# ChuhanZhou/News_Recommendation_Model

Hardware: AMD Instinct MI355X
Metric: train impressions/sec (higher is better)
Workload: dtype f32

## Files before the change

news_recommendation_model_amd/csrc/common.hpp:

```cpp
#pragma once
#include <hip/hip_runtime.h>
#include <stdint.h>

namespace nrm {

using f32x4 = __attribute__((ext_vector_type(4))) float;
using u32x4 = __attribute__((ext_vector_type(4))) unsigned;
using bf16x8 = __attribute__((ext_vector_type(8))) __bf16;

constexpr int WAVE = 64;

inline int device_cus() {
    int dev = 0, cus = 256;
    if (hipGetDevice(&dev) != hipSuccess || hipDeviceGetAttribute(&cus, hipDeviceAttributeMultiprocessorCount, dev) != hipSuccess) cus = 256;
    return cus > 0 ? cus : 256;
}

__device__ __forceinline__ f32x4 mfma16(float a, float b, f32x4 c) {
    return __builtin_amdgcn_mfma_f32_16x16x4f32(a, b, c, 0, 0, 0);
}

struct GeluParts { float cdf; float e; };
__device__ __forceinline__ GeluParts gelu_parts(float x) {
    const float a = fabsf(x) * 0.70710678118654752440f;
    const float t = __builtin_amdgcn_rcpf(fmaf(0.3275911f, a, 1.0f));
    const float e = __builtin_amdgcn_exp2f(-1.44269504088896340736f * a * a);
    float poly = fmaf(1.061405429f, t, -1.453152027f);
    poly = fmaf(poly, t, 1.421413741f);
    poly = fmaf(poly, t, -0.284496736f);
    poly = fmaf(poly, t, 0.254829592f);
    const float half_erfc = 0.5f * poly * t * e;
    GeluParts r;
    r.cdf = x >= 0.f ? 1.0f - half_erfc : half_erfc;
    r.e = e;
    return r;
// ... 61 lines not shown
    v += __shfl_xor(v, 8);
    return v;
}

__device__ __forceinline__ float sum_rows4(float v) {
    const auto a = __builtin_amdgcn_permlane16_swap(__float_as_uint(v), __float_as_uint(v), false, false);
    const float y = __uint_as_float(a[0]) + __uint_as_float(a[1]);
    const auto b = __builtin_amdgcn_permlane32_swap(__float_as_uint(y), __float_as_uint(y), false, false);
    return __uint_as_float(b[0]) + __uint_as_float(b[1]);
}

__device__ __forceinline__ float wave_sum64(float v) {
    v = wave_sum16(v);
    v += __shfl_xor(v, 16);
    v += __shfl_xor(v, 32);
    return v;
}

__device__ __forceinline__ void store_b128_guarded(u32x4 v, __amdgpu_buffer_rsrc_t rs, unsigned voffset, int soffset) {
#if defined(__HIP_DEVICE_COMPILE__)
    __builtin_amdgcn_raw_buffer_store_b128(v, rs, voffset, soffset, 0);
#if !defined(NRM_STORE_GUARD) || NRM_STORE_GUARD == 2
    __builtin_amdgcn_sched_barrier(0);
    asm volatile("s_nop 3");
    __builtin_amdgcn_sched_barrier(0);
#elif NRM_STORE_GUARD == 1
    asm volatile("s_nop 3");
#endif
#endif
}

__host__ __device__ inline int swz4(int row) { return ((row >> 3) & 1) * 3; }

}
```

news_recommendation_model_amd/csrc/gemm.hip:

```cpp
#include <cstdlib>
#include <type_traits>
#include "common.hpp"
#include "gemm.hpp"
#ifndef NRM_PRIO
#define NRM_PRIO 0
#endif
#ifndef NRM_DIAG_GEMM
#define NRM_DIAG_GEMM 0
#endif

namespace nrm {

__global__ void pack_rows_kernel(const float* __restrict__ src, long rs, long cs, int nrows, int ncols,
                                 int rows, int kchunks, float* __restrict__ packed) {
    const long total = (long)kchunks * rows * 16;
    for (long i = (long)blockIdx.x * blockDim.x + threadIdx.x; i < total; i += (long)gridDim.x * blockDim.x) {
        const int j = (int)(i & 15);
        const long rc = i >> 4;
        const int row = (int)(rc % rows);
        const int c = (int)(rc / rows);
        const int slot = (j >> 2) ^ swz4(row);
        const int col = c * 16 + 4 * slot + (j & 3);
        packed[i] = (row < nrows && col < ncols) ? src[row * rs + col * cs] : 0.0f;
    }
}

__global__ __launch_bounds__(256) void pack_rows_multi_kernel(const PackTable tab) {
    const PackEntry e = tab.e[blockIdx.y];
    if (e.fmt) {
        const int nimg = e.fmt;
        const long total = (long)(e.rows / 16) * e.kchunks * 512;
        __bf16* dst = reinterpret_cast<__bf16*>(e.dst);
        for (long i = (long)blockIdx.x * blockDim.x + threadIdx.x; i < total; i += (long)gridDim.x * blockDim.x) {
            const int j = (int)(i & 31), r16 = (int)((i >> 5) & 15);
            const long tc = i >> 9;
            const int c = (int)(tc % e.kchunks), it = (int)(tc / e.kchunks);
            const int n = 16 * it + r16, k = 32 * c + j;
            float v = 0.0f;
            if (n < e.nrows && k < e.ncols) {
                const long o = n * e.rs + k * e.cs;
                v = e.src[o];
// ... 11 lines not shown
        const int j = (int)(i & 15);
        const long rc = i >> 4;
        const int row = (int)(rc % e.rows);
        const int c = (int)(rc / e.rows);
        const int slot = (j >> 2) ^ swz4(row);
        const int col = c * 16 + 4 * slot + (j & 3);
        float v = 0.0f;
        if (row < e.nrows && col < e.ncols) {
            const long o = row * e.rs + col * e.cs;
            v = e.src[o];
            if (e.src2) v = fmaf(e.sign2, e.src2[o], v);
        }
        e.dst[i] = v;
    }
}

hipError_t pack_rows_multi_launch(const PackTable& tab, int n, long max_total, hipStream_t st) {
    if (n <= 0) return hipSuccess;
    long bx = (max_total + 255) / 256;
    if (bx > 128) bx = 128;
    if (bx < 1) bx = 1;
    hipLaunchKernelGGL(pack_rows_multi_kernel, dim3((unsigned)bx, (unsigned)n), dim3(256), 0, st, tab);
    return hipGetLastError();
}

hipError_t pack_rows_launch(const float* src, long rs, long cs, int nrows, int ncols, int rows, int kchunks,
                            float* packed, hipStream_t st) {
    const long total = (long)kchunks * rows * 16;
    const int blocks = (int)((total + 255) / 256 > 4096 ? 4096 : (total + 255) / 256);
    hipLaunchKernelGGL(pack_rows_kernel, dim3(blocks), dim3(256), 0, st, src, rs, cs, nrows, ncols, rows, kchunks, packed);
    return hipGetLastError();
}

template <int NT, int MT, int EPI, int WPE = 2, int KC = 1>
__global__ __launch_bounds__(256, WPE) void gemm_nt_kernel(const GemmNtParams p) {
#if defined(__HIP_DEVICE_COMPILE__)
    constexpr int BM = 4 * MT * 16;
    constexpr int WROWS = NT * 16;
    constexpr int SUB = (WROWS + BM) * 16;
    constexpr int BUF = KC * SUB;
    __shared__ __attribute__((aligned(16))) float smem[2 * BUF];

    const int tid = threadIdx.x;
    const int lane = tid & 63;
    const int wave = __builtin_amdgcn_readfirstlane(tid >> 6);
    const int r16 = lane & 15, q = lane >> 4;
    const int M = p.M;
    const int m0 = blockIdx.x * BM;
    const int nc = blockIdx.y;
    const int n0 = nc * WROWS;

    constexpr unsigned OOB = 0x80000000u;
    const int rows_here = min(BM, M - m0);
    const __amdgpu_buffer_rsrc_t rs_w = __builtin_amdgcn_make_buffer_rsrc(const_cast<float*>(p.wp), 0, p.wp_bytes, 0x00020000);
    const __amdgpu_buffer_rsrc_t rs_x = __builtin_amdgcn_make_buffer_rsrc(
        const_cast<float*>(p.x) + (size_t)m0 * p.ldx, 0, ((rows_here - 1) * p.ldx + p.xcols) * 4, 0x00020000);
    const __amdgpu_buffer_rsrc_t rs_y = __builtin_amdgcn_make_buffer_rsrc(p.y + (size_t)m0 * p.ldy, 0, rows_here * p.ldy * 4, 0x00020000);
    const __amdgpu_buffer_rsrc_t rs_z = __builtin_amdgcn_make_buffer_rsrc(
        p.z ? p.z + (size_t)m0 * p.ldz : nullptr, 0, p.z ? rows_here * p.ldz * 4 : 0, 0x00020000);
    const __amdgpu_buffer_rsrc_t rs_b = __builtin_amdgcn_make_buffer_rsrc(const_cast<float*>(p.bias), 0, p.bias ? (p.N + 3) / 4 * 16 : 0, 0x00020000);
    const __amdgpu_buffer_rsrc_t rs_m = __builtin_amdgcn_make_buffer_rsrc(
        const_cast<float*>(EPI == EPI_MUL ? p.m + (size_t)m0 * p.ldm : nullptr), 0, EPI == EPI_MUL ? rows_here * p.ldm * 4 : 0, 0x00020000);

    unsigned voff_x[MT];
#pragma unroll
    for (int j = 0; j < MT; ++j) {
        const int rl = (wave * MT + j) * 16 + (lane >> 2);
        const unsigned slot = (unsigned)((lane & 3) ^ swz4(lane >> 2));
        voff_x[j] = rl < rows_here ? (unsigned)(rl * p.ldx + 4 * slot) * 4u : OOB;
    }
    const int rslot = 4 * (q ^ swz4(r16));

    f32x4 acc[NT][MT];
#pragma unroll
    for (int it = 0; it < NT; ++it)
#pragma unroll
        for (int jt = 0; jt < MT; ++jt) acc[it][jt] = f32x4{0.f, 0.f, 0.f, 0.f};

    auto dma_chunk = [&](int c, float* buf) {
        const int wbase = (c * p.rows + n0) * 64;
        for (int pc = wave; pc < NT; pc += 4)
            __builtin_amdgcn_raw_ptr_buffer_load_lds(rs_w, (__attribute__((address_space(3))) void*)(buf + pc * 256),
                                                     16, lane * 16, wbase + pc * 1024, 0, 0);
#pragma unroll
        for (int j = 0; j < MT; ++j)
            __builtin_amdgcn_raw_ptr_buffer_load_lds(rs_x, (__attribute__((address_space(3))) void*)(buf + (WROWS + (wave * MT + j) * 16) * 16),
                                                     16, voff_x[j], c * 64, 0, 0);
    };
    auto dma_stage = [&](int s, float* buf) {
#pragma unroll
        for (int k = 0; k < KC; ++k)
            if (KC == 1 || s * KC + k < p.kchunks) dma_chunk(s * KC + k, buf + k * SUB);
    };
    auto compute = [&](const float* buf, auto full, int ntv, int kleft) {
        constexpr bool FULL = decltype(full)::value;
        const float* Xl = buf + WROWS * 16;
        f32x4 pf[MT];
#pragma unroll
        for (int jt = 0; jt < MT; ++jt) pf[jt] = *reinterpret_cast<const f32x4*>(&Xl[((wave * MT + jt) * 16 + r16) * 16 + rslot]);
        if (kleft < 16) {
            asm volatile("");
            const int kl = kleft - 4 * q;
#pragma unroll
            for (int jt = 0; jt < MT; ++jt)
#pragma unroll
                for (int e = 0; e < 4; ++e) pf[jt][e] = e < kl ? pf[jt][e] : 0.f;
        }
        f32x4 af = *reinterpret_cast<const f32x4*>(&buf[r16 * 16 + rslot]);
#pragma unroll
        for (int it = 0; it < NT; ++it) {
            f32x4 afn = af;
            if (it + 1 < NT) afn = *reinterpret_cast<const f32x4*>(&buf[((it + 1) * 16 + r16) * 16 + rslot]);
            if (FULL || it < ntv) {
#pragma unroll
                for (int j = 0; j < 4; ++j)
#pragma unroll
                    for (int jt = 0; jt < MT; ++jt) acc[it][jt] = mfma16(af[j], pf[jt][j], acc[it][jt]);
            }
            __builtin_amdgcn_sched_barrier(0);
            af = afn;
        }
    };

    const int nt_valid = min(NT, (p.N - n0 + 15) >> 4);
    const int nstages = (p.kchunks + KC - 1) / KC;
    dma_stage(0, smem);
    __syncthreads();
    if (NRM_PRIO) __builtin_amdgcn_s_setprio(NRM_PRIO);
    for (int c = 0; c < nstages; ++c) {
        float* cur = smem + (c & 1) * BUF;
        float* nxt = smem + ((c & 1) ^ 1) * BUF;
        if (c + 1 < nstages && !(NRM_DIAG_GEMM & 4)) dma_stage(c + 1, nxt);
#pragma unroll
        for (int k = 0; k < KC; ++k) {
            if (KC > 1 && c * KC + k >= p.kchunks) break;
            const int kleft = p.K - 16 * (c * KC + k);
            if (nt_valid == NT) compute(cur + k * SUB, std::true_type{}, NT, kleft);
            else compute(cur + k * SUB, std::false_type{}, nt_valid, kleft);
        }
        if (!(NRM_DIAG_GEMM & 1)) __syncthreads();
    }
    if (NRM_PRIO) __builtin_amdgcn_s_setprio(0);
    if (NRM_DIAG_GEMM & 2) return;

#pragma unroll
    for (int it = 0; it < NT; ++it) {
        if (it < nt_valid) {
        const int n = n0 + it * 16 + 4 * q;
        const int nb = (n0 + it * 16) * 4;
        f32x4 bb = f32x4{0.f, 0.f, 0.f, 0.f};
        if (EPI != EPI_DGELU && p.bias) {
            bb = __builtin_bit_cast(f32x4, __builtin_amdgcn_raw_buffer_load_b128(rs_b, 16 * q, nb, 0));
#pragma unroll
            for (int e = 0; e < 4; ++e) bb[e] = n + e < p.N ? bb[e] : 0.f;
        }
#pragma unroll
        for (int jt = 0; jt < MT; ++jt) {
            const int rl = (wave * MT + jt) * 16 + r16;
            f32x4 v = acc[it][jt] + bb;
            if (EPI == EPI_BIAS) {
                if (n < p.ldy) store_b128_guarded(__builtin_bit_cast(u32x4, v), rs_y, (unsigned)(rl * p.ldy + 4 * q) * 4u, nb);
            } else if (EPI == EPI_GELU) {
                if (n < p.ldz) store_b128_guarded(__builtin_bit_cast(u32x4, v), rs_z, (unsigned)(rl * p.ldz + 4 * q) * 4u, nb);
                const f32x4 g = gelu4(v);
                if (n < p.ldy) store_b128_guarded(__builtin_bit_cast(u32x4, g), rs_y, (unsigned)(rl * p.ldy + 4 * q) * 4u, nb);
            } else if (EPI == EPI_MUL) {
                if (n < p.ldz) store_b128_guarded(__builtin_bit_cast(u32x4, v), rs_z, (unsigned)(rl * p.ldz + 4 * q) * 4u, nb);
                f32x4 mm = f32x4{0.f, 0.f, 0.f, 0.f};
                if (n < p.ldm) mm = __builtin_bit_cast(f32x4, __builtin_amdgcn_raw_buffer_load_b128(rs_m, (unsigned)(rl * p.ldm + 4 * q) * 4u, nb, 0));
                if (n < p.ldy) store_b128_guarded(__builtin_bit_cast(u32x4, v * mm), rs_y, (unsigned)(rl * p.ldy + 4 * q) * 4u, nb);
            } else {
                f32x4 zz = f32x4{0.f, 0.f, 0.f, 0.f};
                if (n < p.ldz) zz = __builtin_bit_cast(f32x4, __builtin_amdgcn_raw_buffer_load_b128(rs_z, (unsigned)(rl * p.ldz + 4 * q) * 4u, nb, 0));
                const f32x4 g = gelu_grad4_times(zz, acc[it][jt]);
                if (n < p.ldy) store_b128_guarded(__builtin_bit_cast(u32x4, g), rs_y, (unsigned)(rl * p.ldy + 4 * q) * 4u, nb);
            }
        }
        }
        __builtin_amdgcn_sched_barrier(0);
    }
#endif
}

GemmNtPlan gemm_nt_plan(int N) {
    const int n16 = (N + 15) / 16;
    GemmNtPlan pl;
    if (n16 <= 4) { pl.NT = 4; pl.MT = 4; }
    else {
        const int p13 = (n16 + 12) / 13 * 13, p8 = (n16 + 7) / 8 * 8;
        int best = p13 <= p8 ? p13 : p8;
        if (p13 <= p8) { pl.NT = 13; pl.MT = 1; } else { pl.NT = 8; pl.MT = 3; }
        static const bool narrow = [] { const char* e = getenv("NRM_NT_NARROW"); return !(e && e[0] == '0'); }();
        const int p9 = (n16 + 8) / 9 * 9, p5 = (n16 + 4) / 5 * 5;
        if (narrow && p9 * 10 <= best * 9) { pl.NT = 9; pl.MT = 2; best = p9; }
        if (narrow && p5 * 10 <= best * 9) { pl.NT = 5; pl.MT = 4; best = p5; }
    }
    pl.nchunks = (n16 + pl.NT - 1) / pl.NT;
    pl.rows = pl.nchunks * pl.NT * 16;
    return pl;
}

template <int NT, int MT, int WPE = 2, int KC = 1>
static hipError_t launch_nt(const GemmNtParams& p, const GemmNtPlan& pl, int epi, hipStream_t st) {
    constexpr int BM = 4 * MT * 16;
    const dim3 grid((p.M + BM - 1) / BM, pl.nchunks), block(256);
    if (KC > 1) {
        constexpr int lds = 2 * KC * (NT * 16 + BM) * 16 * 4;
        static_assert(lds <= 160 * 1024, "two stages must fit the CU's LDS");
    }
    switch (epi) {
        case EPI_BIAS:  hipLaunchKernelGGL((gemm_nt_kernel<NT, MT, EPI_BIAS, WPE, KC>), grid, block, 0, st, p); break;
        case EPI_GELU:  hipLaunchKernelGGL((gemm_nt_kernel<NT, MT, EPI_GELU, WPE, KC>), grid, block, 0, st, p); break;
        case EPI_DGELU: hipLaunchKernelGGL((gemm_nt_kernel<NT, MT, EPI_DGELU, WPE, KC>), grid, block, 0, st, p); break;
        case EPI_MUL:   hipLaunchKernelGGL((gemm_nt_kernel<NT, MT, EPI_MUL, WPE, KC>), grid, block, 0, st, p); break;
        default: return hipErrorInvalidValue;
    }
    return hipGetLastError();
}

hipError_t gemm_nt_launch(const GemmNtParams& p, const GemmNtPlan& pl, int epi, hipStream_t st) {
    if (p.M <= 0) return hipSuccess;
    static const bool small_m = [] { const char* e = getenv("NRM_NT_SMALLM"); return !(e && e[0] == '0'); }();
    const long wgs = (long)((p.M + 64 * pl.MT - 1) / (64 * pl.MT)) * pl.nchunks;
    const char* kc_e = getenv("NRM_NT_KC");
    int kc = kc_e ? atoi(kc_e) : 1;
    if (kc != 2 && kc != 4) kc = 1;
    if (p.kchunks < 2 * kc) kc = p.kchunks >= 4 ? 2 : 1;
    if (kc > 1 && (pl.MT == 1 || (small_m && wgs < 512))) {
        if (kc == 4) {
            if (pl.NT == 4) return launch_nt<4, 1, 1, 4>(p, pl, epi, st);
            if (pl.NT == 5) return launch_nt<5, 1, 1, 4>(p, pl, epi, st);
            if (pl.NT == 8) return launch_nt<8, 1, 1, 4>(p, pl, epi, st);
            if (pl.NT == 9) return launch_nt<9, 1, 1, 4>(p, pl, epi, st);
            if (pl.NT == 13) return launch_nt<13, 1, 1, 4>(p, pl, epi, st);
        } else {
            if (pl.NT == 4) return launch_nt<4, 1, 2, 2>(p, pl, epi, st);
            if (pl.NT == 5) return launch_nt<5, 1, 2, 2>(p, pl, epi, st);
            if (pl.NT == 8) return launch_nt<8, 1, 2, 2>(p, pl, epi, st);
            if (pl.NT == 9) return launch_nt<9, 1, 2, 2>(p, pl, epi, st);
            if (pl.NT == 13) return launch_nt<13, 1, 2, 2>(p, pl, epi, st);
        }
    }
    if (small_m && pl.MT > 1 && wgs < 512) {
        if (pl.NT == 4) return launch_nt<4, 1, 4>(p, pl, epi, st);
        if (pl.NT == 5) return launch_nt<5, 1, 4>(p, pl, epi, st);
        if (pl.NT == 8) return launch_nt<8, 1, 4>(p, pl, epi, st);
        if (pl.NT == 9) return launch_nt<9, 1, 4>(p, pl, epi, st);
// ... 301 lines not shown
```

news_recommendation_model_amd/csrc/pwattn_bwd_dp.hip:

```cpp
#include <cstdlib>
#ifndef NRM_DIAG_DP
#define NRM_DIAG_DP 0
#endif
#ifndef DP_WPE
#define DP_WPE 3
#endif
#include "common.hpp"
#include "pwattn.hpp"

namespace nrm {

__host__ __device__ inline int dp_tile_col(int NT, int it, int i) {
    const int ng4 = NT >> 2;
    return it < 4 * ng4 ? 64 * (it >> 2) + 4 * i + (it & 3) : 64 * ng4 + 16 * (it - 4 * ng4) + i;
}

__global__ void pack_wpt_f32_kernel(const float* __restrict__ w, int ldw, int D, int NT, int rows, int kchunks,
                                    float* __restrict__ packed) {
    const long total = (long)kchunks * rows * 16;
    for (long i = (long)blockIdx.x * blockDim.x + threadIdx.x; i < total; i += (long)gridDim.x * blockDim.x) {
        const int j = (int)(i & 15);
        const long rc = i >> 4;
        const int row = (int)(rc % rows);
        const int c = (int)(rc / rows);
        const int slot = (j >> 2) ^ swz4(row);
        const int k = c * 16 + 4 * slot + (j & 3);
        const int nc = row / (16 * NT), rr = row - nc * 16 * NT;
        const int d = nc * 16 * NT + dp_tile_col(NT, rr >> 4, rr & 15);
        packed[i] = (k < D && d < D) ? w[(long)k * ldw + d] : 0.0f;
    }
}

BwdDpPlan pwattn_bwd_dp_plan(int D, int H) {
    BwdDpPlan pl = {};
    if (D <= 0 || D % 4 || H < 16) return pl;
    const int n16 = (D + 15) / 16;
    int nch = (n16 + 12) / 13;
    int nt = (n16 + nch - 1) / nch;
    if (nt < 4) nt = 4;
    static const int kNT[4] = {4, 8, 12, 13};
    int sel = 3;
    for (int i = 0; i < 4; ++i) if (kNT[i] >= nt) { sel = i; break; }
    pl.NT = kNT[sel];
    pl.nchunks = (n16 + pl.NT - 1) / pl.NT;
    pl.rows = pl.nchunks * pl.NT * 16;
    pl.kchunks = n16;
    return pl;
}

long pwattn_bwd_dp_packed_floats(int D, int H) {
    const BwdDpPlan pl = pwattn_bwd_dp_plan(D, H);
    return pl.NT ? (long)pl.kchunks * pl.rows * 16 : 0;
}

hipError_t pwattn_bwd_dp_pack_launch(const float* wp, int ldw, int D, int H, float* packed, hipStream_t st) {
    const BwdDpPlan pl = pwattn_bwd_dp_plan(D, H);
    if (!pl.NT) return hipErrorInvalidValue;
    const long total = (long)pl.kchunks * pl.rows * 16;
    const int blocks = (int)((total + 255) / 256 > 2048 ? 2048 : (total + 255) / 256);
    hipLaunchKernelGGL(pack_wpt_f32_kernel, dim3(blocks), dim3(256), 0, st, wp, ldw, D, pl.NT, pl.rows, pl.kchunks, packed);
    return hipGetLastError();
}

template <int NT>
__global__ __launch_bounds__(256, DP_WPE) void bwd_dp_walk_kernel(const BwdDpParams p) {
#if defined(__HIP_DEVICE_COMPILE__)
    constexpr int NW = 4, BM = 64;
    constexpr int WROWS = NT * 16;
    constexpr int NG4 = NT / 4, NREST = NT % 4;
    constexpr int BUF = (WROWS + BM) * 16;
    __shared__ __attribute__((aligned(16))) float smem[2 * BUF + NW * 256];

    const int tid = threadIdx.x;
    const int lane = tid & 63;
    const int wave = __builtin_amdgcn_readfirstlane(tid >> 6);
    const int c16 = lane & 15, q = lane >> 4;
    const int T = p.T, H = p.H, D = p.D, R = p.B * p.H;
    const int KCH = p.kchunks, NCH = p.nchunks;
    float* bounce = smem + 2 * BUF + wave * 256;

    const long S = p.steps;
    const int g = blockIdx.x, G = gridDim.x;
    const int s_lo = (int)(S * g / G), s_hi = (int)(S * (g + 1) / G);
    if (s_lo >= s_hi) return;

    constexpr unsigned OOB = 0x80000000u;
    const __amdgpu_buffer_rsrc_t rs_w = __builtin_amdgcn_make_buffer_rsrc(const_cast<float*>(p.wimg), 0, p.w_bytes, 0x00020000);
    const __amdgpu_buffer_rsrc_t rs_h = __builtin_amdgcn_make_buffer_rsrc(const_cast<float*>(p.h), 0, p.h_bytes, 0x00020000);
    const __amdgpu_buffer_rsrc_t rs_t = __builtin_amdgcn_make_buffer_rsrc(const_cast<float*>(p.t), 0, p.t_bytes, 0x00020000);
    const int rslot = 4 * (q ^ swz4(c16));
    const int zstep = H * D * 4;

    int rb = -1, nc = -1, colbase = 0;
    unsigned live = 0;
    __amdgpu_buffer_rsrc_t rs_z = rs_w;
    unsigned voff_z = OOB;
    unsigned voff_h4[4], voff_h1[4];
// ... 59 lines not shown
                const int dcol = colbase + 64 * gg + lane;
#pragma unroll
                for (int i = 0; i < 4; ++i) {
                    const float v = bounce[i * 64 + lane];
                    const int rw = rw0 + 4 * i + r;
                    if (rw < R && dcol < D) atomicAdd(p.dh + (size_t)rw * D + dcol, v);
                }
            }
        }
#pragma unroll
        for (int i = 0; i < NREST; ++i) {
            const int it = 4 * NG4 + i;
            if (!((live >> it) & 1)) continue;
            const int dcol = colbase + 64 * NG4 + 16 * i + c16;
#pragma unroll
            for (int r = 0; r < 4; ++r) {
                const int rw = rw0 + 4 * q + r;
                if (rw < R && dcol < D) atomicAdd(p.dh + (size_t)rw * D + dcol, dhacc[it][r]);
            }
        }
    };

    auto dma_chunk = [&](int c, int t, float* buf) {
        const int wbase = (c * p.rows + nc * WROWS) * 64;
        if (!((NRM_DIAG_DP & 4) && c > 0))
        for (int pc = wave; pc < NT; pc += NW)
            __builtin_amdgcn_raw_ptr_buffer_load_lds(rs_w, (__attribute__((address_space(3))) void*)(buf + pc * 256),
                                                     16, lane * 16, wbase + pc * 1024, 0, 0);
        if (!((NRM_DIAG_DP & 1) && c > 0))
        __builtin_amdgcn_raw_ptr_buffer_load_lds(rs_z, (__attribute__((address_space(3))) void*)(buf + (WROWS + wave * 16) * 16),
                                                 16, voff_z, t * zstep + c * 64, 0, 0);
    };

    enter(s_lo);
    dma_chunk(0, s_lo % T, smem);
    __syncthreads();
    int par = 0;
    for (int s = s_lo; s < s_hi; ++s) {
        const int t = s % T;
        f32x4 acc[NT];
#pragma unroll
        for (int it = 0; it < NT; ++it) acc[it] = f32x4{0.f, 0.f, 0.f, 0.f};
        const bool more = s + 1 < s_hi;
        const bool same_item = (s + 1) % T != 0;
        for (int c = 0; c < KCH; ++c) {
            float* cur = smem + par * BUF;
            float* nxt = smem + (par ^ 1) * BUF;
            if (c + 1 < KCH) dma_chunk(c + 1, t, nxt);
            else if (more && same_item) dma_chunk(0, t + 1, nxt);
            {
                f32x4 pf = *reinterpret_cast<const f32x4*>(&cur[(WROWS + wave * 16 + c16) * 16 + rslot]);
                if (D - 16 * c < 16) { asm volatile(""); pf = 4 * q < D - 16 * c ? pf : f32x4{0.f, 0.f, 0.f, 0.f}; }
                f32x4 af = *reinterpret_cast<const f32x4*>(&cur[c16 * 16 + rslot]);
#pragma unroll
                for (int it = 0; it < NT; ++it) {
                    f32x4 afn = af;
                    if (it + 1 < NT) afn = *reinterpret_cast<const f32x4*>(&cur[((it + 1) * 16 + c16) * 16 + rslot]);
                    if ((live >> it) & 1)
#pragma unroll
                        for (int j = 0; j < 4; ++j) acc[it] = mfma16(pf[j], af[j], acc[it]);
                    __builtin_amdgcn_sched_barrier(0);
                    af = afn;
                }
            }
            __syncthreads();
            par ^= 1;
        }

        if (NRM_DIAG_DP & 2) {
#pragma unroll
            for (int it = 0; it < NT; ++it) { asm volatile("" :: "v"(acc[it])); dhacc[it] += acc[it]; }
            continue;
        }
        const int soff_h = colbase * 4;
        const int soff_t = (t * D + colbase) * 4;
        float* dtA = p.dt + (rowA + t) * D + colbase;
        float* dtB = dtA + (size_t)T * D;
#pragma unroll
        for (int gg = 0; gg < NG4; ++gg) {
            if (!((live >> (4 * gg)) & 1)) continue;
            f32x4 h4[4];
#pragma unroll
            for (int r = 0; r < 4; ++r)
                h4[r] = __builtin_bit_cast(f32x4, __builtin_amdgcn_raw_buffer_load_b128(rs_h, voff_h4[r], soff_h + 256 * gg, 0));
            const f32x4 tA = __builtin_bit_cast(f32x4, __builtin_amdgcn_raw_buffer_load_b128(rs_t, voff_tA4, soff_t + 256 * gg, 0));
            f32x4 tB = tA;
            if (has_b) tB = __builtin_bit_cast(f32x4, __builtin_amdgcn_raw_buffer_load_b128(rs_t, voff_tB4, soff_t + 256 * gg, 0));
            float xA[4], xB[4];
#pragma unroll
            for (int j = 0; j < 4; ++j) {
                const f32x4 a = acc[4 * gg + j];
                float sa = 0.f, sb = 0.f;
#pragma unroll
// ... 36 lines not shown
            if (has_b) tB = __builtin_bit_cast(float, __builtin_amdgcn_raw_buffer_load_b32(rs_t, voff_tB1, soff_t + so, 0));
            const f32x4 a = acc[it];
            float sa = 0.f, sb = 0.f;
#pragma unroll
            for (int r = 0; r < 4; ++r) {
                const float pr = a[r] * h1[r];
                if (has_b) { sa += isB[r] ? 0.f : pr; sb += isB[r] ? pr : 0.f; }
                else sa += pr;
                dhacc[it][r] = fmaf(a[r], (has_b && isB[r]) ? tB : tA, dhacc[it][r]);
            }
            const int dl = 64 * NG4 + 16 * i + c16;
            const bool dok = colbase + dl < D && q == 0;
            const float vA = sum_rows4(sa);
            if (dok && voff_tA4 != OOB) atomicAdd(dtA + dl, vA);
            if (has_b) {
                const float vB = sum_rows4(sb);
                if (dok) atomicAdd(dtB + dl, vB);
            }
        }

        if (more && !same_item) {
            flush();
            enter(s + 1);
            dma_chunk(0, 0, smem + par * BUF);
            __syncthreads();
        }
    }
    flush();
#endif
}

int pwattn_bwd_dp_diag_flags() { return NRM_DIAG_DP ? 1024 : 0; }

template <int NT>
static hipError_t launch_dp(BwdDpParams p, hipStream_t st) {
    long grid = 12L * device_cus();
    if (const char* e = getenv("NRM_DP_GRID")) { const long v = atol(e); if (v > 0) grid = v; }
    if (grid > p.steps / 4) grid = p.steps / 4;
    if (grid < 1) grid = 1;
    hipLaunchKernelGGL((bwd_dp_walk_kernel<NT>), dim3((unsigned)grid), dim3(256), 0, st, p);
    return hipGetLastError();
}

hipError_t pwattn_bwd_dp_launch(BwdDpParams p, hipStream_t st) {
    const BwdDpPlan pl = pwattn_bwd_dp_plan(p.D, p.H);
    if (!pl.NT) return hipErrorInvalidValue;
    const long R = (long)p.B * p.H;
    const long nrb = (R + 63) / 64;
    p.rows = pl.rows; p.kchunks = pl.kchunks; p.nchunks = pl.nchunks;
    p.steps = nrb * pl.nchunks * p.T;
    if (p.steps <= 0) return hipSuccess;
    if (p.steps > 0x7fffffffL) return hipErrorInvalidValue;
    switch (pl.NT) {
        case 4:  return launch_dp<4>(p, st);
        case 8:  return launch_dp<8>(p, st);
        case 12: return launch_dp<12>(p, st);
        case 13: return launch_dp<13>(p, st);
    }
    return hipErrorInvalidValue;
}

}
```

news_recommendation_model_amd/csrc/pwattn_fwd.hip:

```cpp
#include <cstdlib>
#ifndef XCD_REMAP
#define XCD_REMAP 1
#endif
#ifndef NRM_DIAG_FWD
#define NRM_DIAG_FWD 0
#endif
#ifndef NRM_FWD_NW8
#define NRM_FWD_NW8 0
#endif
#ifndef NRM_PRIO
#define NRM_PRIO 0
#endif
#include "common.hpp"
#include "pwattn.hpp"

namespace nrm {

__global__ void pack_wp_kernel(const float* __restrict__ w, int ldw, int D, int rows, int kchunks,
                               float* __restrict__ packed) {
    const long total = (long)kchunks * rows * 16;
    for (long i = (long)blockIdx.x * blockDim.x + threadIdx.x; i < total; i += (long)gridDim.x * blockDim.x) {
        const int j = (int)(i & 15);
        const long rc = i >> 4;
        const int row = (int)(rc % rows);
        const int c = (int)(rc / rows);
        const int slot = (j >> 2) ^ swz4(row);
        const int d = c * 16 + 4 * slot + (j & 3);
        packed[i] = (row < D && d < D) ? w[(long)row * ldw + d] : 0.0f;
    }
}

template <int NT, int MT, bool SAVE_Z, int WPE = 2, bool CT = false, int NW = 4, bool RAGGED = false, bool HRAG = false>
__global__ __launch_bounds__(NW * 64, WPE) void pwattn_fwd_kernel(const FwdParams p, const RaggedTabs rg) {
#if defined(__HIP_DEVICE_COMPILE__)
    constexpr int BM = NW * MT * 16;
    constexpr int WROWS = NT * 16;
    constexpr int BUF = (WROWS + (CT ? BM + 16 : 2 * BM)) * 16;
    __shared__ __attribute__((aligned(16))) float smem[2 * BUF];

    const int tid = threadIdx.x;
    const int lane = tid & 63;
    const int wave = __builtin_amdgcn_readfirstlane(tid >> 6);
    const int r16 = lane & 15, q = lane >> 4;
    const int M = (int)p.M;
    const int nblk = gridDim.x, lin = blockIdx.x;
    const int xq = nblk >> 3, xr = nblk & 7, xcd = lin & 7;
    const int tile_id = XCD_REMAP ? (xcd < xr ? xcd * (xq + 1) : xr * (xq + 1) + (xcd - xr) * xq) + (lin >> 3) : lin;
    const int m0 = tile_id * BM;
    const int T = p.T, H = p.H, D = p.D;
    const int rows_here = min(BM, M - m0);
    static_assert(!HRAG || (RAGGED && !SAVE_Z && NW * MT <= 16), "history-ragged: a ragged form without z, at most 16 tiles per workgroup");
    auto hrow = [&](int m, unsigned& bt, unsigned& hr) -> bool {
        const int4 e = rg.tile_tab[m >> 4];
        bt = (unsigned)min(max(e.x, 0), rg.N - 1);
        hr = (unsigned)min(max(e.y, 0), rg.R) + (unsigned)(m & 15);
        return (m & 15) < e.z;
    };

    constexpr unsigned OOB = 0x80000000u;
    const __amdgpu_buffer_rsrc_t rs_w = __builtin_amdgcn_make_buffer_rsrc(const_cast<float*>(p.wp), 0, p.wp_bytes, 0x00020000);
    const __amdgpu_buffer_rsrc_t rs_t = __builtin_amdgcn_make_buffer_rsrc(const_cast<float*>(p.t), 0, p.t_bytes, 0x00020000);
    const __amdgpu_buffer_rsrc_t rs_h = __builtin_amdgcn_make_buffer_rsrc(const_cast<float*>(p.h), 0, p.h_bytes, 0x00020000);
    const __amdgpu_buffer_rsrc_t rs_u = __builtin_amdgcn_make_buffer_rsrc(const_cast<float*>(p.u), 0, p.h_bytes, 0x00020000);
    const __amdgpu_buffer_rsrc_t rs_v = __builtin_amdgcn_make_buffer_rsrc(const_cast<float*>(p.v), 0, p.t_bytes, 0x00020000);
    const __amdgpu_buffer_rsrc_t rs_w2 = __builtin_amdgcn_make_buffer_rsrc(const_cast<float*>(p.w2), 0, D * 4, 0x00020000);
// ... 53 lines not shown
            const unsigned b = RAGGED ? (unsigned)min(max(rg.cand_imp[bt], 0), rg.B - 1) : bt / (unsigned)T;
            const unsigned hr = b * H + (mm - bt * H);
            voff_u[jt] = m < M ? (hr * p.ldu + 4 * q) * 4u : OOB;
            voff_v[jt] = m < M ? (bt * p.ldv + 4 * q) * 4u : OOB;
        }
    }
    const int rslot = 4 * (q ^ swz4(r16));

    float s_part[MT];
#pragma unroll
    for (int jt = 0; jt < MT; ++jt) s_part[jt] = 0.f;

    for (int nc = 0; nc < p.nchunks; ++nc) {
        const int kc0 = nc * WROWS;
        const int nt_live = min(NT, (D - kc0 + 15) >> 4);
        f32x4 acc[NT][MT];
#pragma unroll
        for (int jt = 0; jt < MT; ++jt) {
#pragma unroll
            for (int it = 0; it < NT; ++it) {
                const int kb = (kc0 + it * 16) * 4;
                f32x4 uu = f32x4{0.f, 0.f, 0.f, 0.f}, vv = uu;
                if (!(NRM_DIAG_FWD & 1)) {
                    uu = __builtin_bit_cast(f32x4, __builtin_amdgcn_raw_buffer_load_b128(rs_u, voff_u[jt], kb, 0));
                    vv = __builtin_bit_cast(f32x4, __builtin_amdgcn_raw_buffer_load_b128(rs_v, voff_v[jt], kb, 0));
                }
                const bool kok = kc0 + it * 16 + 4 * q < D;
                acc[it][jt] = kok ? uu + vv : f32x4{0.f, 0.f, 0.f, 0.f};
                if ((it & 3) == 3) __builtin_amdgcn_sched_barrier(0);
            }
            __builtin_amdgcn_sched_barrier(0);
        }

        auto dma_chunk = [&](int c, float* buf) {
            const int wbase = (c * p.rows + nc * WROWS) * 64;
            for (int pc = wave; pc < NT; pc += NW)
                __builtin_amdgcn_raw_ptr_buffer_load_lds(rs_w, (__attribute__((address_space(3))) void*)(buf + pc * 256),
                                                         16, lane * 16, wbase + pc * 1024, 0, 0);
#pragma unroll
            for (int j = 0; j < MT; ++j) {
                float* tdst = buf + (WROWS + (wave * MT + j) * 16) * 16;
                if (CT) {
                    __builtin_amdgcn_raw_ptr_buffer_load_lds(rs_h, (__attribute__((address_space(3))) void*)tdst, 16, voff_h[j], c * 64, 0, 0);
                } else {
                    __builtin_amdgcn_raw_ptr_buffer_load_lds(rs_t, (__attribute__((address_space(3))) void*)tdst, 16, voff_t[j], c * 64, 0, 0);
                    __builtin_amdgcn_raw_ptr_buffer_load_lds(rs_h, (__attribute__((address_space(3))) void*)(tdst + BM * 16), 16, voff_h[j], c * 64, 0, 0);
                }
            }
            if (CT && wave == (NT % NW == 0 ? NW - 1 : NT % NW))
                __builtin_amdgcn_raw_ptr_buffer_load_lds(rs_t, (__attribute__((address_space(3))) void*)(buf + (WROWS + BM) * 16), 16, voff_tc, c * 64, 0, 0);
        };
        auto compute = [&](const float* buf, int kleft) {
            const float* Tl = buf + WROWS * 16;
            f32x4 pf[MT];
#pragma unroll
            for (int jt = 0; jt < MT; ++jt) {
                const int ro = ((wave * MT + jt) * 16 + r16) * 16 + rslot;
                if (CT) pf[jt] = *reinterpret_cast<const f32x4*>(&Tl[ro]) * *reinterpret_cast<const f32x4*>(&Tl[BM * 16 + tfrag[jt]]);
                else pf[jt] = *reinterpret_cast<const f32x4*>(&Tl[ro]) * *reinterpret_cast<const f32x4*>(&Tl[BM * 16 + ro]);
            }
            if (kleft < 16) {
                asm volatile("");
#pragma unroll
                for (int jt = 0; jt < MT; ++jt) pf[jt] = 4 * q < kleft ? pf[jt] : f32x4{0.f, 0.f, 0.f, 0.f};
            }
            f32x4 af = *reinterpret_cast<const f32x4*>(&buf[r16 * 16 + rslot]);
#pragma unroll
            for (int it = 0; it < NT; ++it) {
                f32x4 afn = af;
                if (it + 1 < NT) afn = *reinterpret_cast<const f32x4*>(&buf[((it + 1) * 16 + r16) * 16 + rslot]);
                if (WPE < 3 || it < nt_live)
#pragma unroll
                for (int j = 0; j < 4; ++j)
#pragma unroll
                    for (int jt = 0; jt < MT; ++jt) acc[it][jt] = mfma16(af[j], pf[jt][j], acc[it][jt]);
                __builtin_amdgcn_sched_barrier(0);
                af = afn;
            }
        };

        dma_chunk(0, smem);
        __syncthreads();
        if (NRM_PRIO) __builtin_amdgcn_s_setprio(NRM_PRIO);
        for (int c = 0; c < p.kchunks; ++c) {
            float* cur = smem + (c & 1) * BUF;
            float* nxt = smem + ((c & 1) ^ 1) * BUF;
            if (c + 1 < p.kchunks && !((NRM_DIAG_FWD & 2) && c > 0)) dma_chunk(c + 1, nxt);
            compute(cur, D - 16 * c);
            __syncthreads();
        }
        if (NRM_PRIO) __builtin_amdgcn_s_setprio(0);

        f32x4 wq[3];
#pragma unroll
        for (int it = 0; it < 2 && it < NT; ++it)
            wq[it] = __builtin_bit_cast(f32x4, __builtin_amdgcn_raw_buffer_load_b128(rs_w2, 16 * q, (kc0 + it * 16) * 4, 0));
#pragma unroll
        for (int it = 0; it < NT; ++it) {
            const int kb = (kc0 + it * 16) * 4;
            const bool kok = kc0 + it * 16 + 4 * q < D;
            if (it + 2 < NT) wq[(it + 2) % 3] = __builtin_bit_cast(f32x4, __builtin_amdgcn_raw_buffer_load_b128(rs_w2, 16 * q, kb + 128, 0));
            const f32x4 ww = wq[it % 3];
#pragma unroll
            for (int jt = 0; jt < MT; ++jt) {
                const f32x4 zz = acc[it][jt];
                if (SAVE_Z && kok && !(NRM_DIAG_FWD & 4)) {
                    const unsigned vz = (unsigned)(((wave * MT + jt) * 16 + r16) * D + 4 * q) * 4u;
                    store_b128_guarded(__builtin_bit_cast(u32x4, zz), rs_z, vz, kb);
                }
                if (NRM_DIAG_FWD & 8) s_part[jt] += ww[0] * zz[0] + ww[1] * zz[1] + ww[2] * zz[2] + ww[3] * zz[3];
                else s_part[jt] += gelu_dot4(ww, zz);
            }
            __builtin_amdgcn_sched_barrier(0);
        }
    }

    const float b2 = p.b2[0];
#pragma unroll
    for (int jt = 0; jt < MT; ++jt) {
        const float v = sum_rows4(s_part[jt]);
        const int m = m0 + (wave * MT + jt) * 16 + r16;
        if constexpr (HRAG) { if (q == 0 && m < M) p.s[m] = row_ok[jt] ? v + b2 : 0.f; }
        else if (q == 0 && m < M) p.s[m] = v + b2;
    }
#endif
}


static const int kNT[10] = {4, 6, 8, 10, 12, 13, 14, 16, 20, 25};
static const int kMT[10] = {4, 4, 3, 1, 1, 1, 2, 1, 1, 1};

FwdPlan pwattn_fwd_plan(int D) {
    const int n16 = (D + 15) / 16;
    int nch = n16 <= 25 ? 1 : (n16 + 15) / 16;
    static const int use13 = [] { const char* e = getenv("NRM_FWD_13X1"); return e && e[0] == '0' ? 0 : 1; }();
    if (use13 && n16 >= 21 && n16 <= 26) nch = 2;
    const int need = (n16 + nch - 1) / nch;
    int sel = 9;
    for (int i = 0; i < 10; ++i) if (kNT[i] >= need) { sel = i; break; }
    FwdPlan pl;
    pl.NT = kNT[sel]; pl.MT = kMT[sel]; pl.nchunks = nch;
    pl.rows = nch * pl.NT * 16; pl.kchunks = n16;
    return pl;
}

template <int RAGGED, int NT, int MT, int WPE = 2, bool CT = false, int NW = 4>
static hipError_t launch_fwd_t(const FwdParams& p, const RaggedTabs& rg, hipStream_t st) {
    constexpr int BM = NW * MT * 16;
    const long nblk = (p.M + BM - 1) / BM;
    if (nblk <= 0) return hipSuccess;
    if (nblk > 0x7fffffffL) return hipErrorInvalidValue;
    const dim3 grid((unsigned)nblk), block(NW * 64);
    if constexpr (RAGGED == 2) {
        if constexpr (NW * MT <= 16) hipLaunchKernelGGL((pwattn_fwd_kernel<NT, MT, false, WPE, CT, NW, true, true>), grid, block, 0, st, p, rg);
        else return hipErrorInvalidValue;
    }
    else if constexpr (RAGGED == 1) hipLaunchKernelGGL((pwattn_fwd_kernel<NT, MT, false, WPE, CT, NW, true>), grid, block, 0, st, p, rg);
    else if (p.z) hipLaunchKernelGGL((pwattn_fwd_kernel<NT, MT, true, WPE, CT, NW>), grid, block, 0, st, p, rg);
    else          hipLaunchKernelGGL((pwattn_fwd_kernel<NT, MT, false, WPE, CT, NW>), grid, block, 0, st, p, rg);
    return hipGetLastError();
}

static bool fwd_compact_t(int H, int block_rows = 64) {
    const char* e = getenv("NRM_FWD_CT");
    if (e && e[0] == '0') return false;
    if ((block_rows - 1) / H + 2 > 16) return false;
    if (e && e[0] == '1') return true;
    return H >= 16;
}

template <int RAGGED>
static hipError_t fwd_dispatch(const FwdParams& p, const FwdPlan& pl, const RaggedTabs& rg, hipStream_t st) {
#define NRM_FWD(...) launch_fwd_t<RAGGED, __VA_ARGS__>(p, rg, st)
    auto fwd_compact_t = [&](int H, int block_rows = 64) { return RAGGED == 2 ? nrm::fwd_compact_t(rg.k_max >= 16 ? 64 : 1, block_rows) : nrm::fwd_compact_t(H, block_rows); };
    switch (pl.NT) {
        case 4:  return NRM_FWD(4, 4);
        case 6:  return NRM_FWD(6, 4);
        case 8:  return NRM_FWD(8, 3);
        case 10: return fwd_compact_t(p.H) ? NRM_FWD(10, 1, 4, true) : NRM_FWD(10, 1, 3);
        case 12: return fwd_compact_t(p.H) ? NRM_FWD(12, 1, 4, true) : NRM_FWD(12, 1, 3);
        case 13:
            if (!fwd_compact_t(p.H, NRM_FWD_NW8 && !RAGGED ? 128 : 64)) return NRM_FWD(13, 1, 3);
#if NRM_FWD_NW8
            if constexpr (!RAGGED) return NRM_FWD(13, 1, 4, true, 8);
            else
#endif
            return NRM_FWD(13, 1, 4, true);
        case 14: return NRM_FWD(14, 2);
        case 16: return NRM_FWD(16, 1);
        case 20: return NRM_FWD(20, 1);
        case 25: return NRM_FWD(25, 1);
    }
// ... 40 lines not shown
```

Before: 35360.

## Spread next-chunk LDS DMA issues across MFMA tile iterations

Splits the next k-chunk's global-to-LDS buffer loads into per-wave pieces and issues each piece inside the MFMA loop after a chosen output tile. Before, all loads were issued in one burst ahead of compute. The aim is to interleave memory issue with matrix math and smooth VMEM queue pressure. This is on by default for the pwattn forward and backward-dp kernels, and off for gemm (NRM_DMA_PLACE is 0 there). The env var NRM_DMA_SPREAD can turn it off. It adds extra template instantiations and a risk of issue-slot contention inside the compute loop.

```diff
diff --git a/news_recommendation_model_amd/csrc/common.hpp b/news_recommendation_model_amd/csrc/common.hpp
--- a/news_recommendation_model_amd/csrc/common.hpp
+++ b/news_recommendation_model_amd/csrc/common.hpp
@@ -1,6 +1,7 @@
 #pragma once
 #include <hip/hip_runtime.h>
 #include <stdint.h>
+#include <cstdlib>
 
 namespace nrm {
 
@@ -128,4 +129,13 @@
 
 __host__ __device__ inline int swz4(int row) { return ((row >> 3) & 1) * 3; }
 
+constexpr int dma_piece_tile(int place, int i, int nw, int np, int NT) {
+    const int half = (NT + 1) / 2;
+    if (place == 1) return i % half;
+    if (place == 2) return (2 * i) % NT;
+    const int nr = np - nw < half ? np - nw : half;
+    return i >= nw ? (i - nw) % half : (nr + 2 * i) % NT;
 }
+inline bool dma_spread() { const char* e = getenv("NRM_DMA_SPREAD"); return !(e && e[0] == '0'); }
+
+}
diff --git a/news_recommendation_model_amd/csrc/gemm.hip b/news_recommendation_model_amd/csrc/gemm.hip
--- a/news_recommendation_model_amd/csrc/gemm.hip
+++ b/news_recommendation_model_amd/csrc/gemm.hip
@@ -7,6 +7,9 @@
 #endif
 #ifndef NRM_DIAG_GEMM
 #define NRM_DIAG_GEMM 0
+#endif
+#ifndef NRM_DMA_PLACE
+#define NRM_DMA_PLACE 0
 #endif
 
 namespace nrm {
@@ -84,8 +87,9 @@
     return hipGetLastError();
 }
 
-template <int NT, int MT, int EPI, int WPE = 2, int KC = 1>
+template <int NT, int MT, int EPI, int WPE = 2, int KC = 1, int PLACE = 0>
 __global__ __launch_bounds__(256, WPE) void gemm_nt_kernel(const GemmNtParams p) {
+    static_assert(KC == 1 || PLACE == 0, "per-piece DMA issue: one chunk per stage");
 #if defined(__HIP_DEVICE_COMPILE__)
     constexpr int BM = 4 * MT * 16;
     constexpr int WROWS = NT * 16;
@@ -139,12 +143,26 @@
             __builtin_amdgcn_raw_ptr_buffer_load_lds(rs_x, (__attribute__((address_space(3))) void*)(buf + (WROWS + (wave * MT + j) * 16) * 16),
                                                      16, voff_x[j], c * 64, 0, 0);
     };
+    constexpr int NWP = (NT + 3) / 4, NP = NWP + MT;
+    auto dma_piece = [&](int i, int c, float* buf) {
+        if (i < NWP) {
+            const int pc = wave + 4 * i;
+            const int wbase = (c * p.rows + n0) * 64;
+            if (pc < NT)
+                __builtin_amdgcn_raw_ptr_buffer_load_lds(rs_w, (__attribute__((address_space(3))) void*)(buf + pc * 256),
+                                                         16, lane * 16, wbase + pc * 1024, 0, 0);
+        } else {
+            const int j = i - NWP;
+            __builtin_amdgcn_raw_ptr_buffer_load_lds(rs_x, (__attribute__((address_space(3))) void*)(buf + (WROWS + (wave * MT + j) * 16) * 16),
+                                                     16, voff_x[j], c * 64, 0, 0);
+        }
+    };
     auto dma_stage = [&](int s, float* buf) {
 #pragma unroll
         for (int k = 0; k < KC; ++k)
             if (KC == 1 || s * KC + k < p.kchunks) dma_chunk(s * KC + k, buf + k * SUB);
     };
-    auto compute = [&](const float* buf, auto full, int ntv, int kleft) {
+    auto compute = [&](const float* buf, auto full, int ntv, int kleft, bool pre, int cn, float* nxt) {
         constexpr bool FULL = decltype(full)::value;
         const float* Xl = buf + WROWS * 16;
         f32x4 pf[MT];
@@ -168,6 +186,11 @@
                 for (int j = 0; j < 4; ++j)
 #pragma unroll
                     for (int jt = 0; jt < MT; ++jt) acc[it][jt] = mfma16(af[j], pf[jt][j], acc[it][jt]);
+            }
+            if constexpr (PLACE != 0) {
+#pragma unroll
+                for (int i = 0; i < NP; ++i)
+                    if (dma_piece_tile(PLACE, i, NWP, NP, NT) == it && pre) dma_piece(i, cn, nxt);
             }
             __builtin_amdgcn_sched_barrier(0);
             af = afn;
@@ -182,13 +205,14 @@
     for (int c = 0; c < nstages; ++c) {
         float* cur = smem + (c & 1) * BUF;
         float* nxt = smem + ((c & 1) ^ 1) * BUF;
-        if (c + 1 < nstages && !(NRM_DIAG_GEMM & 4)) dma_stage(c + 1, nxt);
+        const bool pre = c + 1 < nstages && !(NRM_DIAG_GEMM & 4);
+        if (PLACE == 0 && pre) dma_stage(c + 1, nxt);
 #pragma unroll
         for (int k = 0; k < KC; ++k) {
             if (KC > 1 && c * KC + k >= p.kchunks) break;
             const int kleft = p.K - 16 * (c * KC + k);
-            if (nt_valid == NT) compute(cur + k * SUB, std::true_type{}, NT, kleft);
-            else compute(cur + k * SUB, std::false_type{}, nt_valid, kleft);
+            if (nt_valid == NT) compute(cur + k * SUB, std::true_type{}, NT, kleft, pre, c + 1, nxt);
+            else compute(cur + k * SUB, std::false_type{}, nt_valid, kleft, pre, c + 1, nxt);
         }
         if (!(NRM_DIAG_GEMM & 1)) __syncthreads();
     }
@@ -252,8 +276,9 @@
     return pl;
 }
 
-template <int NT, int MT, int WPE = 2, int KC = 1>
+template <int NT, int MT, int WPE = 2, int KC = 1, int PLACE = (KC == 1 && !(NT == 8 && MT == 1) ? NRM_DMA_PLACE : 0)>
 static hipError_t launch_nt(const GemmNtParams& p, const GemmNtPlan& pl, int epi, hipStream_t st) {
+    if constexpr (PLACE != 0) if (!dma_spread()) return launch_nt<NT, MT, WPE, KC, 0>(p, pl, epi, st);
     constexpr int BM = 4 * MT * 16;
     const dim3 grid((p.M + BM - 1) / BM, pl.nchunks), block(256);
     if (KC > 1) {
@@ -261,10 +286,10 @@
         static_assert(lds <= 160 * 1024, "two stages must fit the CU's LDS");
     }
     switch (epi) {
-        case EPI_BIAS:  hipLaunchKernelGGL((gemm_nt_kernel<NT, MT, EPI_BIAS, WPE, KC>), grid, block, 0, st, p); break;
-        case EPI_GELU:  hipLaunchKernelGGL((gemm_nt_kernel<NT, MT, EPI_GELU, WPE, KC>), grid, block, 0, st, p); break;
-        case EPI_DGELU: hipLaunchKernelGGL((gemm_nt_kernel<NT, MT, EPI_DGELU, WPE, KC>), grid, block, 0, st, p); break;
-        case EPI_MUL:   hipLaunchKernelGGL((gemm_nt_kernel<NT, MT, EPI_MUL, WPE, KC>), grid, block, 0, st, p); break;
+        case EPI_BIAS:  hipLaunchKernelGGL((gemm_nt_kernel<NT, MT, EPI_BIAS, WPE, KC, PLACE>), grid, block, 0, st, p); break;
+        case EPI_GELU:  hipLaunchKernelGGL((gemm_nt_kernel<NT, MT, EPI_GELU, WPE, KC, PLACE>), grid, block, 0, st, p); break;
+        case EPI_DGELU: hipLaunchKernelGGL((gemm_nt_kernel<NT, MT, EPI_DGELU, WPE, KC, PLACE>), grid, block, 0, st, p); break;
+        case EPI_MUL:   hipLaunchKernelGGL((gemm_nt_kernel<NT, MT, EPI_MUL, WPE, KC, PLACE>), grid, block, 0, st, p); break;
         default: return hipErrorInvalidValue;
     }
     return hipGetLastError();
diff --git a/news_recommendation_model_amd/csrc/pwattn_bwd_dp.hip b/news_recommendation_model_amd/csrc/pwattn_bwd_dp.hip
--- a/news_recommendation_model_amd/csrc/pwattn_bwd_dp.hip
+++ b/news_recommendation_model_amd/csrc/pwattn_bwd_dp.hip
@@ -4,6 +4,9 @@
 #endif
 #ifndef DP_WPE
 #define DP_WPE 3
+#endif
+#ifndef NRM_DMA_PLACE
+#define NRM_DMA_PLACE 1
 #endif
 #include "common.hpp"
 #include "pwattn.hpp"
@@ -62,7 +65,7 @@
     return hipGetLastError();
 }
 
-template <int NT>
+template <int NT, int PLACE = 0>
 __global__ __launch_bounds__(256, DP_WPE) void bwd_dp_walk_kernel(const BwdDpParams p) {
 #if defined(__HIP_DEVICE_COMPILE__)
     constexpr int NW = 4, BM = 64;
@@ -188,6 +191,20 @@
                                                  16, voff_z, t * zstep + c * 64, 0, 0);
     };
 
+    constexpr int NWP = (NT + NW - 1) / NW, NP = NWP + 1;
+    auto dma_piece = [&](int i, int c, int t, float* buf) {
+        if (i < NWP) {
+            const int pc = wave + NW * i;
+            const int wbase = (c * p.rows + nc * WROWS) * 64;
+            if (pc < NT && !((NRM_DIAG_DP & 4) && c > 0))
+                __builtin_amdgcn_raw_ptr_buffer_load_lds(rs_w, (__attribute__((address_space(3))) void*)(buf + pc * 256),
+                                                         16, lane * 16, wbase + pc * 1024, 0, 0);
+        } else if (!((NRM_DIAG_DP & 1) && c > 0)) {
+            __builtin_amdgcn_raw_ptr_buffer_load_lds(rs_z, (__attribute__((address_space(3))) void*)(buf + (WROWS + wave * 16) * 16),
+                                                     16, voff_z, t * zstep + c * 64, 0, 0);
+        }
+    };
+
     enter(s_lo);
     dma_chunk(0, s_lo % T, smem);
     __syncthreads();
@@ -202,8 +219,10 @@
         for (int c = 0; c < KCH; ++c) {
             float* cur = smem + par * BUF;
             float* nxt = smem + (par ^ 1) * BUF;
-            if (c + 1 < KCH) dma_chunk(c + 1, t, nxt);
-            else if (more && same_item) dma_chunk(0, t + 1, nxt);
+            const bool wrap = c + 1 == KCH;
+            const bool pre = !wrap || (more && same_item);
+            const int cn = wrap ? 0 : c + 1, tn = wrap ? t + 1 : t;
+            if (PLACE == 0 && pre) dma_chunk(cn, tn, nxt);
             {
                 f32x4 pf = *reinterpret_cast<const f32x4*>(&cur[(WROWS + wave * 16 + c16) * 16 + rslot]);
                 if (D - 16 * c < 16) { asm volatile(""); pf = 4 * q < D - 16 * c ? pf : f32x4{0.f, 0.f, 0.f, 0.f}; }
@@ -215,6 +234,11 @@
                     if ((live >> it) & 1)
 #pragma unroll
                         for (int j = 0; j < 4; ++j) acc[it] = mfma16(pf[j], af[j], acc[it]);
+                    if constexpr (PLACE != 0) {
+#pragma unroll
+                        for (int i = 0; i < NP; ++i)
+                            if (dma_piece_tile(PLACE, i, NWP, NP, NT) == it && pre) dma_piece(i, cn, tn, nxt);
+                    }
                     __builtin_amdgcn_sched_barrier(0);
                     af = afn;
                 }
@@ -317,13 +341,14 @@
 
 int pwattn_bwd_dp_diag_flags() { return NRM_DIAG_DP ? 1024 : 0; }
 
-template <int NT>
+template <int NT, int PLACE = NRM_DMA_PLACE>
 static hipError_t launch_dp(BwdDpParams p, hipStream_t st) {
+    if constexpr (PLACE != 0) if (!dma_spread()) return launch_dp<NT, 0>(p, st);
     long grid = 12L * device_cus();
     if (const char* e = getenv("NRM_DP_GRID")) { const long v = atol(e); if (v > 0) grid = v; }
     if (grid > p.steps / 4) grid = p.steps / 4;
     if (grid < 1) grid = 1;
-    hipLaunchKernelGGL((bwd_dp_walk_kernel<NT>), dim3((unsigned)grid), dim3(256), 0, st, p);
+    hipLaunchKernelGGL((bwd_dp_walk_kernel<NT, PLACE>), dim3((unsigned)grid), dim3(256), 0, st, p);
     return hipGetLastError();
 }
 
diff --git a/news_recommendation_model_amd/csrc/pwattn_fwd.hip b/news_recommendation_model_amd/csrc/pwattn_fwd.hip
--- a/news_recommendation_model_amd/csrc/pwattn_fwd.hip
+++ b/news_recommendation_model_amd/csrc/pwattn_fwd.hip
@@ -10,6 +10,9 @@
 #endif
 #ifndef NRM_PRIO
 #define NRM_PRIO 0
+#endif
+#ifndef NRM_DMA_PLACE
+#define NRM_DMA_PLACE 1
 #endif
 #include "common.hpp"
 #include "pwattn.hpp"
@@ -30,7 +33,7 @@
     }
 }
 
-template <int NT, int MT, bool SAVE_Z, int WPE = 2, bool CT = false, int NW = 4, bool RAGGED = false, bool HRAG = false>
+template <int NT, int MT, bool SAVE_Z, int WPE = 2, bool CT = false, int NW = 4, bool RAGGED = false, bool HRAG = false, int PLACE = 0>
 __global__ __launch_bounds__(NW * 64, WPE) void pwattn_fwd_kernel(const FwdParams p, const RaggedTabs rg) {
 #if defined(__HIP_DEVICE_COMPILE__)
     constexpr int BM = NW * MT * 16;
@@ -150,25 +153,36 @@
             __builtin_amdgcn_sched_barrier(0);
         }
 
+        constexpr int NWP = (NT + NW - 1) / NW, NRP = CT ? MT : 2 * MT, NP = NWP + NRP + (CT ? 1 : 0);
+        auto dma_piece = [&](int i, int c, float* buf) {
+            if (i < NWP) {
+                const int pc = wave + NW * i;
+                const int wbase = (c * p.rows + nc * WROWS) * 64;
+                if (pc < NT)
+                    __builtin_amdgcn_raw_ptr_buffer_load_lds(rs_w, (__attribute__((address_space(3))) void*)(buf + pc * 256),
+                                                             16, lane * 16, wbase + pc * 1024, 0, 0);
+            } else if (i < NWP + NRP) {
+                const int j = CT ? i - NWP : (i - NWP) >> 1;
+                float* tdst = buf + (WROWS + (wave * MT + j) * 16) * 16;
+                if (CT)
+                    __builtin_amdgcn_raw_ptr_buffer_load_lds(rs_h, (__attribute__((address_space(3))) void*)tdst, 16, voff_h[j], c * 64, 0, 0);
+                else if (((i - NWP) & 1) == 0)
+                    __builtin_amdgcn_raw_ptr_buffer_load_lds(rs_t, (__attribute__((address_space(3))) void*)tdst, 16, voff_t[j], c * 64, 0, 0);
+                else
+                    __builtin_amdgcn_raw_ptr_buffer_load_lds(rs_h, (__attribute__((address_space(3))) void*)(tdst + BM * 16), 16, voff_h[j], c * 64, 0, 0);
+            } else if (wave == (NT % NW == 0 ? NW - 1 : NT % NW)) {
+                __builtin_amdgcn_raw_ptr_buffer_load_lds(rs_t, (__attribute__((address_space(3))) void*)(buf + (WROWS + BM) * 16), 16, voff_tc, c * 64, 0, 0);
+            }
+        };
         auto dma_chunk = [&](int c, float* buf) {
             const int wbase = (c * p.rows + nc * WROWS) * 64;
             for (int pc = wave; pc < NT; pc += NW)
                 __builtin_amdgcn_raw_ptr_buffer_load_lds(rs_w, (__attribute__((address_space(3))) void*)(buf + pc * 256),
                                                          16, lane * 16, wbase + pc * 1024, 0, 0);
 #pragma unroll
-            for (int j = 0; j < MT; ++j) {
-                float* tdst = buf + (WROWS + (wave * MT + j) * 16) * 16;
-                if (CT) {
-                    __builtin_amdgcn_raw_ptr_buffer_load_lds(rs_h, (__attribute__((address_space(3))) void*)tdst, 16, voff_h[j], c * 64, 0, 0);
-                } else {
-                    __builtin_amdgcn_raw_ptr_buffer_load_lds(rs_t, (__attribute__((address_space(3))) void*)tdst, 16, voff_t[j], c * 64, 0, 0);
-                    __builtin_amdgcn_raw_ptr_buffer_load_lds(rs_h, (__attribute__((address_space(3))) void*)(tdst + BM * 16), 16, voff_h[j], c * 64, 0, 0);
-                }
-            }
-            if (CT && wave == (NT % NW == 0 ? NW - 1 : NT % NW))
-                __builtin_amdgcn_raw_ptr_buffer_load_lds(rs_t, (__attribute__((address_space(3))) void*)(buf + (WROWS + BM) * 16), 16, voff_tc, c * 64, 0, 0);
+            for (int i = NWP; i < NP; ++i) dma_piece(i, c, buf);
         };
-        auto compute = [&](const float* buf, int kleft) {
+        auto compute = [&](const float* buf, int kleft, bool pre, int cn, float* nxt) {
             const float* Tl = buf + WROWS * 16;
             f32x4 pf[MT];
 #pragma unroll
@@ -192,6 +206,11 @@
                 for (int j = 0; j < 4; ++j)
 #pragma unroll
                     for (int jt = 0; jt < MT; ++jt) acc[it][jt] = mfma16(af[j], pf[jt][j], acc[it][jt]);
+                if constexpr (PLACE != 0) {
+#pragma unroll
+                    for (int i = 0; i < NP; ++i)
+                        if (dma_piece_tile(PLACE, i, NWP, NP, NT) == it && pre) dma_piece(i, cn, nxt);
+                }
                 __builtin_amdgcn_sched_barrier(0);
                 af = afn;
             }
@@ -203,8 +222,9 @@
         for (int c = 0; c < p.kchunks; ++c) {
             float* cur = smem + (c & 1) * BUF;
             float* nxt = smem + ((c & 1) ^ 1) * BUF;
-            if (c + 1 < p.kchunks && !((NRM_DIAG_FWD & 2) && c > 0)) dma_chunk(c + 1, nxt);
-            compute(cur, D - 16 * c);
+            const bool pre = c + 1 < p.kchunks && !((NRM_DIAG_FWD & 2) && c > 0);
+            if (PLACE == 0 && pre) dma_chunk(c + 1, nxt);
+            compute(cur, D - 16 * c, pre, c + 1, nxt);
             __syncthreads();
         }
         if (NRM_PRIO) __builtin_amdgcn_s_setprio(0);
@@ -262,20 +282,21 @@
     return pl;
 }
 
-template <int RAGGED, int NT, int MT, int WPE = 2, bool CT = false, int NW = 4>
+template <int RAGGED, int NT, int MT, int WPE = 2, bool CT = false, int NW = 4, int PLACE = NRM_DMA_PLACE>
 static hipError_t launch_fwd_t(const FwdParams& p, const RaggedTabs& rg, hipStream_t st) {
+    if constexpr (PLACE != 0) if (!dma_spread()) return launch_fwd_t<RAGGED, NT, MT, WPE, CT, NW, 0>(p, rg, st);
     constexpr int BM = NW * MT * 16;
     const long nblk = (p.M + BM - 1) / BM;
     if (nblk <= 0) return hipSuccess;
     if (nblk > 0x7fffffffL) return hipErrorInvalidValue;
     const dim3 grid((unsigned)nblk), block(NW * 64);
     if constexpr (RAGGED == 2) {
-        if constexpr (NW * MT <= 16) hipLaunchKernelGGL((pwattn_fwd_kernel<NT, MT, false, WPE, CT, NW, true, true>), grid, block, 0, st, p, rg);
+        if constexpr (NW * MT <= 16) hipLaunchKernelGGL((pwattn_fwd_kernel<NT, MT, false, WPE, CT, NW, true, true, PLACE>), grid, block, 0, st, p, rg);
         else return hipErrorInvalidValue;
     }
-    else if constexpr (RAGGED == 1) hipLaunchKernelGGL((pwattn_fwd_kernel<NT, MT, false, WPE, CT, NW, true>), grid, block, 0, st, p, rg);
-    else if (p.z) hipLaunchKernelGGL((pwattn_fwd_kernel<NT, MT, true, WPE, CT, NW>), grid, block, 0, st, p, rg);
-    else          hipLaunchKernelGGL((pwattn_fwd_kernel<NT, MT, false, WPE, CT, NW>), grid, block, 0, st, p, rg);
+    else if constexpr (RAGGED == 1) hipLaunchKernelGGL((pwattn_fwd_kernel<NT, MT, false, WPE, CT, NW, true, false, PLACE>), grid, block, 0, st, p, rg);
+    else if (p.z) hipLaunchKernelGGL((pwattn_fwd_kernel<NT, MT, true, WPE, CT, NW, false, false, PLACE>), grid, block, 0, st, p, rg);
+    else          hipLaunchKernelGGL((pwattn_fwd_kernel<NT, MT, false, WPE, CT, NW, false, false, PLACE>), grid, block, 0, st, p, rg);
     return hipGetLastError();
 }
 
```

Result: no change. 35680 (median of 6 runs) (+0.9%).
